# SamsungLabs/Metis

Hardware: NVIDIA B200
Metric: candidate plans evaluated/sec (higher is better)
Workload: dtype f64

## Files before the change

metis_b200/csrc/metis_coop.cuh:

```cuda
#pragma once

#include "metis_eval.cuh"

#ifdef METIS_HOST_STATS
extern "C" void metis_host_stats(int slot, long add);
#endif

namespace metis {

struct CoopMail {
    int m;
    int err;
    int flag;
    int pad;
    double val;
    double val2;
    int k;
    int s_top;
    int top_skip;
    int pad2;
};

struct OneLane {
    bool reverse = false;
// ... 605 lines not shown
                owner[layer] = (uint8_t)top;
                w.capa[top] = ntop;
                w.capa[nb] = nnb;
                if (top > nb) { int r = layer - 1; while (owner[r] != nb) --r; w.lastl[nb] = (uint16_t)r; }
                else          { int r = layer + 1; while (owner[r] != nb) ++r; w.first[nb] = (uint16_t)r; }
                if (w.cnt[top] == 0) { w.first[top] = (uint16_t)layer; w.lastl[top] = (uint16_t)layer; }
                else {
                    if (layer < (int)w.first[top]) w.first[top] = (uint16_t)layer;
                    if (layer > (int)w.lastl[top]) w.lastl[top] = (uint16_t)layer;
                }
                ++w.cnt[top];
                --w.cnt[nb];
            }
            x.sync();
        }
        x.mark(16);
        int carry = 0;
#pragma unroll 1
        for (int base = 0; base < S; base += x.width()) {
            const int s = base + x.lane();
            const int v = s < S ? (int)w.cnt[s] : 0;
            const int inc = x.incl_scan(v);
            if (s < S) w.part[s + 1] = (uint16_t)(carry + inc);
            carry += x.last_lane(inc);
        }
        if (x.leader()) w.part[0] = 0;
        x.sync();
        return METIS_FATAL_NONE;
    }

    MB_HD int adjust_performance_coop() {
        const int S = pd.S;
        const bool one_type = ONE || T.p.num_types == 1;
        double *ratio = reinterpret_cast<double *>(w.subw);
        double *mcap = ratio + MAXS / 2;
        static_assert(MAXL >= MAXS, "subw doubles as two S-sized fp64 arrays only when MAXL >= 2 * MAXS / 2");
        (void)mcap;
        x.sync();
        METIS_PAR(x, s, S) {
            const int a = one_type ? 0 : this->rank_start(s), b = a + this->group(s);
            const double c = w.perf[s], md = w.extra[s];
            const double mc = one_type ? T.type_memory[0] * (double)this->group(s) : this->memory_capacity(a, b);
            double av, adj;
            if (mc > md) {
                adj = c;
                av = (c * mc / md) - c;
            } else {
                av = 0.0;
                adj = c * (mc / md) * 0.9;
            }
            w.capa[s] = av;
            w.mstate[s] = adj;
            ratio[s] = (mc > md) ? 0.0 : (c - adj);
        }
        x.sync();
        if (x.leader()) {
            double need = 0.;
#pragma unroll 4
            for (int s = 0; s < S; ++s)
                if (w.capa[s] == 0.0 && ratio[s] != 0.0) need += ratio[s];
                else if (ratio[s] != 0.0) need += ratio[s];
            mail.val = need;
            mail.flag = seq_py_sum(w.capa, S) < need ? 1 : 0;
        }
        x.sync();
        if (mail.flag) return 1;
        METIS_PAR(x, s, S) w.extra[s] = 0.;
        x.sync();
        if (x.leader()) {
            double need = mail.val;
// ... 53 lines not shown
                const int rc = this->hetero_memory_demand(s, type0, md);
                if (rc) err = (double)rc + (double)aux * 256.0;
            }
            const double state = one_type ? T.type_memory[0] * (double)(1 << g) - md : this->memory_capacity(a, b) - md;
            w.extra[s] = md;
            w.capa[s] = state;
            w.mstate[s] = err;
            failed = failed || err != 0.0;
            oom = oom || state < 0;
        }
        failed = x.any(failed);
        oom = x.any(oom);
        if (failed) return -first_error(w.mstate, S);
        x.sync();
        if (!oom) {
            METIS_PAR(x, s, S) w.mstate[s] = w.capa[s];
            x.sync();
            return 1;
        }
        if (attempt >= 3) return 0;
        x.mark(21);
        const int rc = adjust_performance_coop();
        if (rc < 0) return rc;
        return rc == 1 ? 0 : 2;
    }

    MB_HD int get_cost_coop(double &cost_out) {
        const int per = T.p.devices_per_node;
        const int Lm = T.p.num_layers;
        const bool one_type = ONE || T.p.num_types == 1;
        const bool ubw = T.p.uniform_bw != 0;
        const int nstage = pd.label < pd.S ? pd.label : pd.S;
        if (T.p.q10_devices < T.p.total_devices && this->rank_start(nstage) > T.p.q10_devices) return 1;
        double *ppterm = reinterpret_cast<double *>(w.subw);
        bool bad = false;
        double max_len = -INFINITY, max_upd = -INFINITY, max_dp = -INFINITY;
        x.sync();
        METIS_PAR(x, s, nstage) {
            const int g = w.gcode[s], tpc = w.tpc[s];
            const int a = one_type ? 0 : this->rank_start(s), b = a + (1 << g);
            const int la = w.part[s], lb = w.part[s + 1];
            const int ldp = g - tpc;
            const int mbs = bs_total >> ldp;
            const int ta = one_type ? 0 : type_of_rank(T, pd.ns, a);
            const int tb = one_type ? 0 : type_of_rank(T, pd.ns, b - 1);
            double len = 0.0;
            if (ta == tb) {
                const int key = key_of(T, ta, tpc, mbs);
                if (key < 0) bad = true;
                else len = range_sum<SerialUniform>(T, kRangeLc, key, T.lc + (size_t)key * T.p.lpad, la, lb);
            } else if (this->hetero_exec_cost(a, b, 1 << ldp, tpc, la, lb, len)) {
                bad = true;
            }
            w.capa[s] = len;
            if (len > max_len) max_len = len;
            const double inv_tp = pow2_neg(tpc);
            double pp = 0.0;
            if (s < nstage - 1) {
                if (ubw) {
                    pp = (lb == Lm - 1) ? T.pp_vocab[mbs * T.p.num_tp + tpc] : T.pp_hidden[mbs];
                } else {
                    double act;
                    if (lb == Lm - 1)
                        act = (double)((int64_t)mbs * T.p.sequence_length * T.p.vocab_size) * inv_tp;
                    else
                        act = (double)((int64_t)mbs * T.p.sequence_length * T.p.hidden_size);
                    const int a2 = this->rank_start(s), b2 = this->rank_start(s + 2);
// ... 108 lines not shown
```

metis_b200/csrc/metis_eval.cuh:

```cuda
#pragma once

#include <stdint.h>
#include <string.h>
#include <math.h>

#include "../../include/metis_b200.h"

#if defined(__CUDACC__)
#define MB_HD __host__ __device__ __forceinline__
#define MB_HD_NOINLINE __host__ __device__ __noinline__
#else
#define MB_HD inline
#define MB_HD_NOINLINE inline
#endif

namespace metis {

template <class V>
MB_HD V list_load(const V *p) {
#if defined(__CUDA_ARCH__)
    return __ldcg(p);
#else
    return *p;
#endif
// ... 114 lines not shown
    unsigned mask;
    __device__ Lockstep() : mask(0xFFFFFFFFu) {}
    __device__ void converge() const { __syncwarp(mask); }
    __device__ void rejoin(bool p) { mask = __ballot_sync(0xFFFFFFFFu, p); }
};
#endif
struct SerialUniform : Serial {
    static constexpr bool kUniform = true;
};

constexpr uint64_t kOnes = 0x0101010101010101ULL;

constexpr uint16_t kBroke = 0x8000;
constexpr uint16_t kTaken = 0x4000;
constexpr uint16_t kPos = 0x3FFF;

template <int MAXS, int MAXL>
struct Scratch {
    static constexpr int kBlock = MAXS + 64;
    double perf[MAXS];
    double capa[MAXS];
    double mstate[MAXS];
    double extra[MAXS];
    uint16_t fe[MAXS];
    uint16_t first[MAXS], lastl[MAXS], cnt[MAXS];
    uint16_t part[MAXS + 1];
    uint16_t rs[MAXS + 1];
    uint8_t gcode[MAXS];
    uint8_t tpc[MAXS];
    uint8_t lstk[MAXS];
    uint8_t got[MAXS];
    uint8_t blk[kBlock];
    uint64_t ownerw[MAXL / 8 + 1];
    uint64_t subw[MAXL];
};

MB_HD double py_sum_range(const double *x, int a, int b) {
    if (a >= b) return 0.0;
    double f = 0.0 + x[a];
    double c = 0.0;
    for (int i = a + 1; i < b; ++i) {
        const double v = x[i];
        const double t = f + v;
        if (fabs(f) >= fabs(v)) c += (f - t) + v;
        else c += (v - t) + f;
        f = t;
    }
    if (c != 0.0 && isfinite(c)) f += c;
    return f;
}

MB_HD_NOINLINE double py_sum_range_compact(const double *x, int a, int b) {
    if (a >= b) return 0.0;
    double f = 0.0 + x[a];
    double c = 0.0;
#pragma unroll 1
    for (int i = a + 1; i < b; ++i) {
        const double v = x[i];
        const double t = f + v;
        if (fabs(f) >= fabs(v)) c += (f - t) + v;
        else c += (v - t) + f;
        f = t;
    }
    if (c != 0.0 && isfinite(c)) f += c;
    return f;
}

// ... 78 lines not shown
#pragma unroll 1
    for (int k = 0; k < nt; ++k)
        if (rank < end[k]) return typ[k];
    return typ[nt - 1];
}

MB_HD int type_of_q10(const Tables &T, int ns, int idx) {
    const int nt = T.p.num_types;
    const int32_t *end = T.q10_end + ns * nt;
    const uint8_t *typ = T.run_type + ns * nt;
#pragma unroll 1
    for (int k = 0; k < nt; ++k)
        if (idx < end[k]) return typ[k];
    return typ[nt - 1];
}

MB_HD int key_of(const Tables &T, int type, int tpc, int bs) {
    if (tpc >= T.p.num_tp || bs < 1 || bs > T.p.num_bs) return -1;
    return T.key_index[(type * T.p.num_tp + tpc) * T.p.num_bs + (bs - 1)];
}

template <int MAXS, int MAXL>
MB_HD int fwd_start(const Scratch<MAXS, MAXL> &w, int s) {
    if (s == 0) return 0;
    const uint16_t e = w.fe[s - 1];
    return (e & kPos) + ((e & kBroke) ? 1 : 0);
}

template <int MAXS, int MAXL>
MB_HD bool fwd_nonempty(const Scratch<MAXS, MAXL> &w, int s) {
    return (int)(w.fe[s] & kPos) > fwd_start(w, s);
}

MB_HD void sub_store(uint64_t *subw, int j, int stage) {
    reinterpret_cast<uint8_t *>(subw)[(j / kH) * 8 + (j % kH)] = (uint8_t)stage;
}

MB_HD int popc64(uint64_t v) {
#if defined(__CUDA_ARCH__)
    return __popcll(v);
#else
    return __builtin_popcountll(v);
#endif
}
MB_HD int ctz64(uint64_t v) {
#if defined(__CUDA_ARCH__)
    return __ffsll((long long)v) - 1;
#else
    return __builtin_ctzll(v);
#endif
}
MB_HD int popc32(uint32_t v) {
#if defined(__CUDA_ARCH__)
    return __popc(v);
#else
    return __builtin_popcount(v);
#endif
}
MB_HD int ctz32(uint32_t v) {
#if defined(__CUDA_ARCH__)
    return __ffs((int)v) - 1;
#else
    return __builtin_ctz(v);
#endif
}
MB_HD int clz32(uint32_t v) {
#if defined(__CUDA_ARCH__)
    return __clz((int)v);
#else
    return __builtin_clz(v);
// ... 31 lines not shown
    const int c0 = (int)(v & 0xFF), c1 = (int)((v >> 8) & 0xFF), c2 = (int)((v >> 16) & 0xFF);
    if (swar_count(v, c0) * 2 > kH) return c0;
    if (c1 != c0 && swar_count(v, c1) * 2 > kH) return c1;
    if (c2 != c1 && c2 != c0 && swar_count(v, c2) * 2 > kH) return c2;
    return (int)kDropped;
}

template <int MAXS, int MAXL, class X>
MB_HD int balance_run(const Tables &T, int S, Scratch<MAXS, MAXL> &w, const X &x) {
    const int L = T.p.num_layers;
    if (T.p.norm_len < L) return METIS_FATAL_INDEX;
    const double *dlay = T.dlay;
    const double *lc = T.norm_lc;
    const int N = kH * L;
    const int lim = (N - 1 - kH) > 0 ? (N - 1 - kH) : 0;
    const int last = S - 1;
    int broken = METIS_FATAL_NONE;

    x.sync();
#pragma unroll (X::kUniform ? 1 : 0)
    for (int s = x.lane(); s < S; s += x.width()) { w.capa[s] = w.perf[s]; w.got[s] = 0; w.cnt[s] = 0; }
    x.sync();

    x.mark(10);
    int k = 0, sTop = -1;
    bool topSkip = false;
    if (S > 1) {
        int s = 0, j = 0;
        double c = w.capa[0];
#pragma unroll (X::kUniform ? 1 : 0)
        for (int r = 0; r + 1 < L; ++r) {
            const double d = dlay[r];
            const int nsub = (r == L - 2) ? kH - 1 : kH;
            const int s_in = s;
            uint64_t v = 0;
#pragma unroll
            for (int q = 0; q < kH; ++q) {
                if (q < nsub) {
                    if (s < last) {
                        if (c > d) {
                            c -= d;
                            v |= (uint64_t)(uint32_t)s << (8 * q);
                        } else {
                            w.capa[s] = c;
                            w.fe[s] = (uint16_t)(j | kBroke);
                            ++s;
                            c = w.capa[s];
                        }
                    }
                    ++j;
                }
            }
            if (s_in < last) w.subw[r] = v;
        }
        if (s < last) {
            w.capa[s] = c;
            w.fe[s] = (uint16_t)lim;
#pragma unroll (X::kUniform ? 1 : 0)
            for (int t = s + 1; t < last; ++t) w.fe[t] = (uint16_t)lim;
            k = lim;
            sTop = s;
        } else {
            k = (w.fe[last - 1] & kPos) + 1;
            sTop = last - 1;
            topSkip = true;
        }
    }

    x.mark(11);
    x.converge();
    int m;
    {
        double c = w.capa[last];
        const double dl = dlay[L - 1];
#pragma unroll (X::kUniform ? 1 : 0)
        for (int i = 0; i < kH; ++i) c -= dl;
        m = N - kH;
        int sp = S - 2;
#pragma unroll (X::kUniform ? 1 : 0)
        while (m > 0) {
            const int j = m - 1;
            bool un = (j >= k);
            if (!un) {
#pragma unroll (X::kUniform ? 1 : 0)
                while (sp >= 0 && (!(w.fe[sp] & kBroke) || (int)(w.fe[sp] & kPos) > j)) --sp;
                un = (sp >= 0 && (int)(w.fe[sp] & kPos) == j);
// ... 19 lines not shown
            const int next_start = pos + ((e & kBroke) ? 1 : 0);
            if ((e & (kBroke | kTaken)) != kBroke) { start = next_start; continue; }
            const int j = pos;
            int lo = 0;
            if (pos > start) {
                lo = s;
            } else {
#pragma unroll (X::kUniform ? 1 : 0)
                for (int u = s;; --u) {
                    if (u < s) {
                        const int t = w.lstk[u];
                        const bool above = (t == last) || (fwd_nonempty(w, t) && fwd_start(w, t) > j);
                        if (!above) { lo = t; break; }
                    }
                    if (fwd_nonempty(w, u)) { lo = u; break; }
                    if (u == 0) break;
                }
            }
            int hi = s + 1;
            if (hi < last && !((int)(w.fe[hi] & kPos) > next_start && !w.got[hi])) {
                ++hi;
#pragma unroll (X::kUniform ? 1 : 0)
                while (hi < last && (!fwd_nonempty(w, hi) || w.got[hi])) ++hi;
            }
            if (lo > hi) { broken = METIS_FATAL_SCRATCH; hi = lo; }
            int pick = lo;
            double best = w.capa[lo];
#pragma unroll (X::kUniform ? 1 : 0)
            for (int t = lo + 1; t <= hi; ++t)
                if (w.capa[t] > best) { best = w.capa[t]; pick = t; }
            w.capa[pick] -= dlay[j / kH];
            w.lstk[s] = (uint8_t)pick;
            w.got[pick] = 1;
            sub_store(w.subw, j, pick);
            start = next_start;
        }
    }
    x.converge();
    int nblk = m - k;
    if (nblk > Scratch<MAXS, MAXL>::kBlock) { broken = METIS_FATAL_SCRATCH; nblk = Scratch<MAXS, MAXL>::kBlock; }
    {
        int below = -1;
#pragma unroll (X::kUniform ? 1 : 0)
        for (int t = 0; t < nblk; ++t) {
            const int j = k + t;
            int lo = 0;
            if (below >= 0) lo = below;
            else if (sTop >= 0) {
#pragma unroll (X::kUniform ? 1 : 0)
                for (int u = sTop;; --u) {
                    if (u < sTop || topSkip) {
                        const uint16_t eu = w.fe[u];
                        if ((eu & (kBroke | kTaken)) == kBroke) {
                            const int t2 = w.lstk[u];
                            if (t2 != last) { lo = t2; break; }
                        }
                    }
                    if (fwd_nonempty(w, u)) { lo = u; break; }
                    if (u == 0) break;
                }
            }
            int pick = lo;
            double best = w.capa[lo];
#pragma unroll (X::kUniform ? 1 : 0)
            for (int t2 = lo + 1; t2 <= last; ++t2)
                if (w.capa[t2] > best) { best = w.capa[t2]; pick = t2; }
            w.capa[pick] -= dlay[j / kH];
            w.blk[t] = (uint8_t)pick;
            if (pick != last) below = pick;
            sub_store(w.subw, j, pick);
        }
    }

    x.mark(13);
    x.converge();
    x.sync();
    int run_own = (int)kDropped, run_first = 0, run_len = 0;
#pragma unroll (X::kUniform ? 1 : 0)
    for (int r = x.lane(); r < L; r += x.width()) {
        const int nlow = m - kH * r;
        int own;
        if (nlow <= 0) {
            own = last;
        } else {
            uint64_t v = w.subw[r];
            if (nlow < kH) {
                const uint64_t mask = (1ULL << (8 * nlow)) - 1ULL;
                v = (v & mask) | (((uint64_t)last * kOnes) & ~mask);
            }
            v |= 0xFF00000000000000ULL;
            own = layer_owner(v, (T.p.corrected & METIS_FIX_Q5) != 0);
        }
        reinterpret_cast<uint8_t *>(w.ownerw)[r] = (uint8_t)own;
        {
            if (own == run_own) ++run_len;
            else {
                if (run_own != (int)kDropped) {
                    if (w.cnt[run_own] == 0) w.first[run_own] = (uint16_t)run_first;
                    w.lastl[run_own] = (uint16_t)(r - 1);
                    w.cnt[run_own] = (uint16_t)(w.cnt[run_own] + run_len);
                }
                run_own = own; run_first = r; run_len = 1;
            }
        }
    }
    if (run_own != (int)kDropped) {
        if (w.cnt[run_own] == 0) w.first[run_own] = (uint16_t)run_first;
        w.lastl[run_own] = (uint16_t)(L - 1);
        w.cnt[run_own] = (uint16_t)(w.cnt[run_own] + run_len);
    }
    x.sync();
    x.mark(14);
    x.converge();
    uint8_t *owner = reinterpret_cast<uint8_t *>(w.ownerw);
    x.sync();
#pragma unroll (X::kUniform ? 1 : 0)
    for (int s = x.lane(); s < S; s += x.width())
        w.capa[s] = w.cnt[s] ? w.perf[s] - range_sum<X>(T, kRangeNorm, 0, lc, w.first[s], (int)w.lastl[s] + 1) : w.perf[s];
    x.sync();

    x.mark(15);
    x.converge();
#pragma unroll (X::kUniform ? 1 : 0)
// ... 353 lines not shown
            if (key < 0) { aux = ((uint32_t)tpc << 16) | (uint32_t)bs; return METIS_FATAL_KEY_MEMORY; }
            demand += range_sum<SerialUniform>(T, kRangeMem, key, T.mem + (size_t)key * T.p.lpad, la, lb) * kMemCoef;
            return 0;
        }
        HSplit hs;
        const int rc = partition_data(T, pd.ns, a, b - a, 1 << (g - tpc), tpc, bs_total, hs, aux);
        if (rc) return rc;
        double worst = 0.0;
#pragma unroll 1
        for (int r = 0; r < hs.nruns; ++r)
#pragma unroll 1
            for (int v = 0; v < 2; ++v) {
                const int cntv = v ? hs.plus[r] : hs.n[r] - hs.plus[r];
                const int h = hs.base[r] + v;
                if (cntv <= 0 || h == 0) continue;
                double need = 0.0;
#pragma unroll 1
                for (int bit = 30; bit >= 0; --bit) {
                    const int piece = 1 << bit;
                    if (!(h & piece)) continue;
                    const int key = key_of(T, hs.type[r], tpc, piece);
                    if (key < 0) { aux = ((uint32_t)tpc << 16) | (uint32_t)piece; return METIS_FATAL_KEY_MEMORY; }
                    need += range_sum<SerialUniform>(T, kRangeMem, key, T.mem + (size_t)key * T.p.lpad, la, lb) * kMemCoef;
                }
                if (need > worst) worst = need;
            }
        demand += worst;
        return 0;
    }

    MB_HD_NOINLINE int adjust_performance() {
        const int S = pd.S;
        const bool one_type = ONE || T.p.num_types == 1;
        double *ratio = reinterpret_cast<double *>(w.subw);
        x.sync();
#pragma unroll (X::kUniform ? 1 : 0)
        for (int s = x.lane(); s < S; s += x.width()) {
            const int a = one_type ? 0 : rank_start(s), b = a + group(s);
            const double c = w.perf[s], md = w.extra[s];
            const double mc = one_type ? T.type_memory[0] * (double)group(s) : memory_capacity(a, b);
            double av, adj;
            if (mc > md) {
                adj = c;
                av = (c * mc / md) - c;
            } else {
                av = 0.0;
                adj = c * (mc / md) * 0.9;
            }
            w.capa[s] = av;
            w.mstate[s] = adj;
        }
        x.sync();
        double need = 0.;
        PySum avail_sum;
#pragma unroll (X::kUniform ? 1 : 0)
        for (int s = 0; s < S; ++s) {
            const int a = one_type ? 0 : rank_start(s);
            const double mc = one_type ? T.type_memory[0] * (double)group(s) : memory_capacity(a, a + group(s));
            if (!(mc > w.extra[s])) need += (w.perf[s] - w.mstate[s]);
            avail_sum.add(w.capa[s]);
        }
        if (avail_sum.result() < need) return 1;
        x.sync();
#pragma unroll (X::kUniform ? 1 : 0)
        for (int s = x.lane(); s < S; s += x.width()) w.extra[s] = 0.;
        x.sync();
        int guard = 0;
// ... 192 lines not shown

    MB_HD int get_cost(double &cost_out) {
        const int per = T.p.devices_per_node;
        const int Lm = T.p.num_layers;
        const bool one_type = ONE || T.p.num_types == 1;
        const bool ubw = T.p.uniform_bw != 0;
        const int nstage = pd.label < pd.S ? pd.label : pd.S;
        if (T.p.q10_devices < T.p.total_devices && rank_start(nstage) > T.p.q10_devices) return 1;
        x.sync();
#pragma unroll (X::kUniform ? 1 : 0)
        for (int s = x.lane(); s < nstage; s += x.width()) {
            const int g = w.gcode[s], tpc = w.tpc[s];
            const int a = one_type ? 0 : rank_start(s), b = a + (1 << g);
            const int la = w.part[s], lb = w.part[s + 1];
            const int ldp = g - tpc;
            const int ta = one_type ? 0 : type_of_rank(T, pd.ns, a);
            const int tb = one_type ? 0 : type_of_rank(T, pd.ns, b - 1);
            double len = 0.0, err = 0.0;
            if (ta == tb) {
                const int key = key_of(T, ta, tpc, bs_total >> ldp);
                if (key < 0) err = 1.0;
                else len = range_sum<X>(T, kRangeLc, key, T.lc + (size_t)key * T.p.lpad, la, lb);
            } else if (hetero_exec_cost(a, b, 1 << ldp, tpc, la, lb, len)) {
                err = 1.0;
            }
            w.capa[s] = len;
            w.extra[s] = err;
        }
        x.sync();
        bool bad = false;
#pragma unroll (X::kUniform ? 1 : 0)
        for (int s = x.lane(); s < nstage; s += x.width()) bad = bad || (w.extra[s] != 0.0);
        if (x.any(bad)) return 1;
        double *ppterm = reinterpret_cast<double *>(w.subw);
        double max_len = -INFINITY, max_upd = -INFINITY, max_dp = -INFINITY;
#pragma unroll (X::kUniform ? 1 : 0)
        for (int s = x.lane(); s < nstage; s += x.width()) {
            const int g = w.gcode[s], tpc = w.tpc[s];
            const int la = w.part[s], lb = w.part[s + 1];
            const int ldp = g - tpc;
            const int mbs = bs_total >> ldp;
            const double inv_tp = pow2_neg(tpc);
            if (w.capa[s] > max_len) max_len = w.capa[s];
            double pp = 0.0;
            if (s < nstage - 1) {
                if (ubw) {
                    pp = (lb == Lm - 1) ? T.pp_vocab[mbs * T.p.num_tp + tpc] : T.pp_hidden[mbs];
                } else {
                    double act;
                    if (lb == Lm - 1)
                        act = (double)((int64_t)mbs * T.p.sequence_length * T.p.vocab_size) * inv_tp;
                    else
                        act = (double)((int64_t)mbs * T.p.sequence_length * T.p.hidden_size);
                    const int a = rank_start(s), b2 = rank_start(s + 2);
                    pp = act / (bw_of_node_range(a / per, (b2 - 1) / per) * 1048576.0);
                }
            }
            ppterm[s] = pp;
            int ntr = lb - la;
            double params = 0.0;
            if (la == 0) { params += T.p.input_params * inv_tp; --ntr; }
            if (lb == Lm) { params += T.p.output_params * inv_tp; --ntr; }
            params += T.p.transformer_params * inv_tp * (double)ntr;
            double dpc;
            if (ubw) dpc = T.dpk[ldp] * params;
            else {
                const int dp = 1 << ldp;
// ... 185 lines not shown
```

metis_b200/csrc/metis_search.cu:

```cuda
#include <cuda_runtime.h>
#include <cooperative_groups.h>
#include <stdint.h>
#include <stdio.h>
#include <stdlib.h>
#include <string.h>

#include "metis_eval.cuh"
#include "metis_coop.cuh"
#include "metis_trace.cuh"
#include "metis_rows.cuh"

namespace cg = cooperative_groups;

namespace metis {

#ifndef METIS_THREADS
#define METIS_THREADS 256
#endif
#ifndef METIS_MIN_BLOCKS
#define METIS_MIN_BLOCKS 3
#endif
#ifndef METIS_MIN_BLOCKS_BIG
#define METIS_MIN_BLOCKS_BIG METIS_MIN_BLOCKS
#endif
#ifndef METIS_MIN_BLOCKS_BIG_ONE
#define METIS_MIN_BLOCKS_BIG_ONE (METIS_MIN_BLOCKS + 1)
#endif
constexpr int kThreads = METIS_THREADS;
constexpr int kMaxS = METIS_MAX_STAGES;
constexpr int kMaxL = METIS_MAX_LAYERS;
constexpr int kSmemBlobMax = 160 * 1024;

static thread_local char g_err[256] = "";
static thread_local cudaEvent_t g_ev_before = nullptr, g_ev_after = nullptr;

static int cuda_fail(cudaError_t e, const char *what) {
    snprintf(g_err, sizeof(g_err), "%s: %s", what, cudaGetErrorString(e));
    return METIS_E_CUDA;
}
static int arg_fail(const char *what) {
    snprintf(g_err, sizeof(g_err), "%s", what);
    return METIS_E_ARG;
}
int fail_cuda(cudaError_t e, const char *what) { return cuda_fail(e, what); }
int fail_arg(const char *what) { return arg_fail(what); }

struct BlobLayout {
    uint32_t total;
    uint32_t key, lc, mem, exec_full, fb, norm, derived, tmem, bwf, bwm, runt, rune, q10e;
    uint32_t rsum, rsum_bytes;
};

static uint32_t align16(uint32_t v) { return (v + 15u) & ~15u; }

static BlobLayout make_layout(const MetisProblem &p) {
    BlobLayout l;
    uint32_t o = 0;
    const uint32_t nkey = (uint32_t)p.num_types * p.num_tp * p.num_bs;
    l.key = o;       o = align16(o + nkey * 2);
    l.lc = o;        o = align16(o + (uint32_t)p.num_keys * p.lpad * 8);
    l.mem = o;       o = align16(o + (uint32_t)p.num_keys * p.lpad * 8);
// ... 3 lines not shown
    l.derived = o;   o = align16(o + (uint32_t)derived_layout(p).total * 8);
    l.tmem = o;      o = align16(o + (uint32_t)p.num_types * 8);
    l.bwf = o;       o = align16(o + (uint32_t)p.num_types * 8);
    l.bwm = o;       o = align16(o + (uint32_t)p.num_types * 8);
    l.runt = o;      o = align16(o + (uint32_t)p.num_node_sequences * p.num_types);
    l.rune = o;      o = align16(o + (uint32_t)p.num_node_sequences * p.num_types * 4);
    l.q10e = o;      o = align16(o + (uint32_t)p.num_node_sequences * p.num_types * 4);
    l.total = o;
    const uint64_t n = (uint64_t)p.num_layers + 1;
    l.rsum = (o + 127u) & ~127u;
    l.rsum_bytes = (uint32_t)((uint64_t)(2 * p.num_keys + 1) * n * n * 8);
    return l;
}

__device__ __forceinline__ Tables make_tables(const MetisProblem &p, const BlobLayout &l, const uint8_t *base,
                                              const uint8_t *gblob = nullptr) {
    Tables T;
    T.p = p;
    T.rsum = gblob ? reinterpret_cast<const double *>(gblob + l.rsum) : nullptr;
    T.key_index = reinterpret_cast<const int16_t *>(base + l.key);
    T.lc = reinterpret_cast<const double *>(base + l.lc);
    T.mem = reinterpret_cast<const double *>(base + l.mem);
    T.exec_full = reinterpret_cast<const double *>(base + l.exec_full);
    T.fb_sync = reinterpret_cast<const double *>(base + l.fb);
    T.norm_lc = reinterpret_cast<const double *>(base + l.norm);
    bind_derived(T, reinterpret_cast<const double *>(base + l.derived));
    T.type_memory = reinterpret_cast<const double *>(base + l.tmem);
    T.bw_first = reinterpret_cast<const double *>(base + l.bwf);
    T.bw_min = reinterpret_cast<const double *>(base + l.bwm);
    T.run_type = base + l.runt;
    T.run_end = reinterpret_cast<const int32_t *>(base + l.rune);
    T.q10_end = reinterpret_cast<const int32_t *>(base + l.q10e);
    return T;
}

__device__ __forceinline__ void copy_bytes(uint8_t *dst, const void *src, uint32_t n, uint32_t tid, uint32_t nthr) {
    const uint8_t *s = static_cast<const uint8_t *>(src);
    for (uint32_t i = tid; i < n; i += nthr) dst[i] = s[i];
}

__global__ void pack_tables_kernel(MetisProblem p, BlobLayout l, uint8_t *blob) {
    const uint32_t tid = blockIdx.x * blockDim.x + threadIdx.x, nthr = gridDim.x * blockDim.x;
    const uint32_t nkey = (uint32_t)p.num_types * p.num_tp * p.num_bs;
    copy_bytes(blob + l.key, p.key_index, nkey * 2, tid, nthr);
    copy_bytes(blob + l.lc, p.layer_compute, (uint32_t)p.num_keys * p.lpad * 8, tid, nthr);
    copy_bytes(blob + l.mem, p.layer_memory, (uint32_t)p.num_keys * p.lpad * 8, tid, nthr);
    copy_bytes(blob + l.exec_full, p.exec_full, (uint32_t)p.num_keys * 8, tid, nthr);
    copy_bytes(blob + l.fb, p.fb_sync, (uint32_t)p.num_keys * 8, tid, nthr);
    copy_bytes(blob + l.norm, p.norm_lc, (uint32_t)p.norm_len * 8, tid, nthr);
    copy_bytes(blob + l.tmem, p.type_memory, (uint32_t)p.num_types * 8, tid, nthr);
    copy_bytes(blob + l.bwf, p.type_bw_first, (uint32_t)p.num_types * 8, tid, nthr);
    copy_bytes(blob + l.bwm, p.type_bw_min, (uint32_t)p.num_types * 8, tid, nthr);
    copy_bytes(blob + l.runt, p.ns_run_type, (uint32_t)p.num_node_sequences * p.num_types, tid, nthr);
    copy_bytes(blob + l.rune, p.ns_run_end, (uint32_t)p.num_node_sequences * p.num_types * 4, tid, nthr);
    copy_bytes(blob + l.q10e, p.ns_q10_end, (uint32_t)p.num_node_sequences * p.num_types * 4, tid, nthr);
    double *derived = reinterpret_cast<double *>(blob + l.derived);
    const DerivedLayout d = derived_layout(p);
    for (uint32_t i = tid; i < (uint32_t)d.total; i += nthr)
        derived[i] = derive_entry(p, d, p.norm_lc, p.exec_full, p.type_bw_first, (int)i);
}

__global__ void __launch_bounds__(128)
range_sums_kernel(MetisProblem p, BlobLayout l, uint8_t *blob) {
    const int L = p.num_layers;
    const long long i = (long long)blockIdx.x * blockDim.x + threadIdx.x;
    if (i >= (long long)range_sum_tables(p) * L) return;
// ... 237 lines not shown
        if (lane == __ffs(peers) - 1) atomicAdd(&ls.ctl[kCtlHist + k], (unsigned int)__popc(peers));
        if (lane == __ffs(peers3) - 1) atomicAdd(&ls.ctl[kCtlHist3 + key], (unsigned int)__popc(peers3));
    }
}

__global__ void __launch_bounds__(256)
het_scatter_kernel(const SearchLists ls) {
    __shared__ unsigned int s_base[160];
    const unsigned int n = ls.ctl[0];
    const bool bulk = (long long)n >= ls.bulk_min;
    const int hist = bulk ? kCtlHist : kCtlHist3, cursor = bulk ? kCtlCursor : kCtlCursor3;
    if (threadIdx.x == 0) {
        unsigned int acc = 0;
        for (int k = 127; k >= 0; --k) { s_base[k] = acc; acc += ls.ctl[hist + k]; }
    }
    __syncthreads();
    const long long span = (long long)gridDim.x * blockDim.x;
    const long long upto = (((long long)n + 31) / 32) * 32;
    for (long long pos = (long long)blockIdx.x * blockDim.x + threadIdx.x; pos < upto; pos += span) {
        const bool live = pos < (long long)n;
        uint4 e = make_uint4(0, 0, 0, 0);
        if (live) e = ls.a[pos];
        const int k = !live ? -1 : bulk ? (int)(e.w & 0xFF) : (int)((e.y >> 8) & 0x7F);
        const unsigned int peers = __match_any_sync(0xFFFFFFFFu, k);
        const int leader = __ffs(peers) - 1, me = threadIdx.x & 31;
        unsigned int at = 0;
        if (live && me == leader) at = atomicAdd(&ls.ctl[cursor + k], (unsigned int)__popc(peers));
        at = __shfl_sync(0xFFFFFFFFu, at, leader);
        if (live) ls.b[(long long)s_base[k] + at + __popc(peers & ((1u << me) - 1u))] = e;
    }
}

template <int MAXS, int MAXL, bool ONE>
__global__ void __launch_bounds__(kThreads, (MAXS <= 64 ? METIS_MIN_BLOCKS : ONE ? METIS_MIN_BLOCKS_BIG_ONE : METIS_MIN_BLOCKS_BIG))
het_first_kernel(const __grid_constant__ MetisProblem p, const __grid_constant__ MetisPlanSpace sp,
                 const __grid_constant__ BlobLayout lay, const uint8_t *__restrict__ blob, const int use_smem,
                 const __grid_constant__ DeviceOut out, const SearchLists ls, const int best_slot) {
    extern __shared__ __align__(128) uint8_t smem[];
    __shared__ uint64_t mbar;
    DeviceSink sink(out);
    const unsigned int n = ls.ctl[0];
    if ((long long)n >= ls.bulk_min) {
        const uint8_t *base = blob;
        if (use_smem) {
            stage_blob_tma(smem, blob, lay.total, &mbar);
            base = smem;
        }
        const Tables T = make_tables(p, lay, base, blob);
        Scratch<MAXS, MAXL> w;
        const int lane = threadIdx.x & 31;
        for (;;) {
            unsigned int fetched = 0;
            if (lane == 0) fetched = atomicAdd(&ls.ctl[1], 1u);
            const long long b0 = 32LL * __shfl_sync(0xFFFFFFFFu, fetched, 0);
            if (b0 >= (long long)n) break;
            const long long pos = b0 + lane;
            PlanDesc pd;
            const bool has = pos < (long long)n;
            uint4 e = make_uint4(0, 0, 0, 0);
            if (has) { e = ls.b[pos]; decode_entry(sp, e, pd); }
            int hint = 0, start = 1;
            const bool cont = first_task<MAXS, MAXL, ONE, Lockstep>(T, w, sink, has, pd, hint, start);
            const unsigned m = __ballot_sync(0xFFFFFFFFu, cont);
            if (m) {
                const int leader = __ffs(m) - 1;
                unsigned int at = 0;
                if (lane == leader) at = atomicAdd(&ls.ctl[2], (unsigned int)__popc(m));
                at = __shfl_sync(0xFFFFFFFFu, at, leader);
                if (cont) {
                    const unsigned key = hint < 0 ? 0u : (hint > 127 ? 127u : (unsigned)hint);
                    const unsigned int c = at + __popc(m & ((1u << lane) - 1u));
                    if (start == 2) {
                        if (c < ls.save_cap) {
                            for (int s = 0; s < pd.S; ++s) ls.perf[(size_t)s * ls.save_cap + c] = w.perf[s];
                        } else start = 1;
                    }
                    e.y = 1u | ((unsigned)start << 1) | (key << 8);
                    ls.a[c] = e;
                    atomicAdd(&ls.ctl[kCtlHist2 + key], 1u);
                }
            }
        }
    }
    finish_block(sink, out, best_slot + blockIdx.x);
}

__global__ void __launch_bounds__(256)
het_order_kernel(const SearchLists ls) {
    __shared__ unsigned int s_base[128];
    if ((long long)ls.ctl[0] < ls.bulk_min) return;
    const unsigned int n = ls.ctl[2];
    if (threadIdx.x == 0) {
        unsigned int acc = 0;
        for (int k = 127; k >= 0; --k) { s_base[k] = acc; acc += ls.ctl[kCtlHist2 + k]; }
    }
    __syncthreads();
    const long long span = (long long)gridDim.x * blockDim.x;
    for (long long pos = (long long)blockIdx.x * blockDim.x + threadIdx.x; pos < (long long)n; pos += span) {
        const uint4 e = ls.a[pos];
        const unsigned key = (e.y >> 8) & 0x7Fu;
        const unsigned int to = s_base[key] + atomicAdd(&ls.ctl[kCtlCursor2 + key], 1u);
        ls.b[to] = e;
        ls.src[to] = (unsigned int)pos;
    }
}

#ifdef METIS_PROFILE_PHASES
__device__ long long g_mark_acc[64];
#endif
struct WarpCoop {
#ifdef METIS_PROFILE_PHASES
// ... 91 lines not shown
        return dkey_inv(kmax(dkey(v), mine));
    }
    __device__ __noinline__ int incl_scan(int v) const {
        const int lane = threadIdx.x & 31;
#pragma unroll
        for (int d = 1; d < 32; d <<= 1) {
            const int u = __shfl_up_sync(0xFFFFFFFFu, v, d);
            if (lane >= d) v += u;
        }
        return v;
    }
    __device__ int last_lane(int v) const { return __shfl_sync(0xFFFFFFFFu, v, 31); }
};

template <int MAXS, int MAXL>
struct alignas(16) ChainScratch {
    Scratch<MAXS, MAXL> w;
    CoopMail mail;
};

template <int MAXS, int MAXL, bool ONE>
__global__ void __launch_bounds__(512, 2)
het_chain_kernel(const __grid_constant__ MetisProblem p, const __grid_constant__ MetisPlanSpace sp,
                 const __grid_constant__ BlobLayout lay, const uint8_t *__restrict__ blob, const int use_smem,
                 const unsigned int scratch_off, const __grid_constant__ DeviceOut out, const SearchLists ls,
                 const int best_slot) {
    extern __shared__ __align__(128) uint8_t smem[];
    __shared__ uint64_t mbar;
    const uint8_t *base = blob;
    if (use_smem) {
        stage_blob_tma(smem, blob, lay.total, &mbar);
        base = smem;
    }
    const Tables T = make_tables(p, lay, base, blob);
    DeviceSink sink(out);
    const int lane = threadIdx.x & 31;
    sink.leader = lane == 0;
    ChainScratch<MAXS, MAXL> *cs = reinterpret_cast<ChainScratch<MAXS, MAXL> *>(smem + scratch_off) + (threadIdx.x >> 5);
    const unsigned int n_adm = ls.ctl[0];
    const bool bulk = (long long)n_adm >= ls.bulk_min;
    const uint4 *list = ls.b;
    const unsigned int n = bulk ? ls.ctl[2] : n_adm;
    WarpCoop lanes;
    CoopEvaluator<MAXS, MAXL, WarpCoop, ONE> ev(T, cs->w, cs->mail, lanes);
    for (;;) {
        unsigned int i = 0;
        if (lane == 0) i = atomicAdd(&ls.ctl[3], 1u);
        i = __shfl_sync(0xFFFFFFFFu, i, 0);
        if (i >= n) break;
        const uint4 e = __ldcg(&list[i]);
        PlanDesc pd;
        decode_entry(sp, e, pd);
        lanes.mark(1);
        const int start = (e.y & 1u) ? (int)((e.y >> 1) & 3u) : 0;
        const double *perf = nullptr;
        if (start == 2) perf = ls.perf + __ldcg(&ls.src[i]);
        ev.run_chain(pd, sink, start, perf, (size_t)ls.save_cap);
        lanes.mark(0);
    }
    while (WarpCoop::block_or(0)) {}
    sink.leader = true;
    if (lane != 0) { sink.n_part = sink.n_run = sink.n_key = 0; }
    finish_block(sink, out, best_slot + blockIdx.x);
}

__global__ void het_finalize_kernel(const MetisRecord *block_best, int nblocks, const unsigned long long *counters,
                                    const unsigned int *ctl, MetisSearchSummary *summary) {
// ... 294 lines not shown
        int best_warps = 0;
        for (int threads = 64; threads <= 512; threads *= 2) {
            if (forced && threads != ((forced + 31) & ~31)) continue;
            const unsigned int off = chain_smem_tables ? blob_pad : 0u;
            const size_t dyn = off + (size_t)(threads / 32) * per_warp;
            if (dyn > (size_t)smem_optin) continue;
            if (dyn > 48 * 1024) {
                e = cudaFuncSetAttribute(chain, cudaFuncAttributeMaxDynamicSharedMemorySize, (int)dyn);
                if (e != cudaSuccess) { cudaGetLastError(); continue; }
            }
            int per_sm = 0;
            e = cudaOccupancyMaxActiveBlocksPerMultiprocessor(&per_sm, chain, threads, dyn);
            if (e != cudaSuccess || per_sm < 1) { cudaGetLastError(); continue; }
            const int warps = per_sm * threads / 32;
            if (warps > best_warps) { best_warps = warps; chain_threads = threads; chain_per_sm = per_sm; chain_dyn = dyn; chain_off = off; }
        }
        if (chain_threads == 0) chain_smem_tables = 0;
    }
    if (chain_threads == 0) return arg_fail("chain kernel does not fit this device (shared memory)");
    if (chain_dyn > 48 * 1024) {
        e = cudaFuncSetAttribute(chain, cudaFuncAttributeMaxDynamicSharedMemorySize, (int)chain_dyn);
        if (e != cudaSuccess) return cuda_fail(e, "cudaFuncSetAttribute(chain)");
    }
    int64_t chain_grid = (int64_t)sms * chain_per_sm;

    auto first = het_first_kernel<MAXS, MAXL, ONE>;
    int first_smem_tables = (int)lay.total <= blob_max && blob_pad <= (unsigned int)smem_optin;
    size_t first_dyn = first_smem_tables ? blob_pad : 0;
    if (first_dyn > 48 * 1024) {
        e = cudaFuncSetAttribute(first, cudaFuncAttributeMaxDynamicSharedMemorySize, (int)first_dyn);
        if (e != cudaSuccess) { cudaGetLastError(); first_smem_tables = 0; first_dyn = 0; }
    }
    int first_per_sm = 0;
    e = cudaOccupancyMaxActiveBlocksPerMultiprocessor(&first_per_sm, first, kThreads, first_dyn);
    if (e != cudaSuccess || first_per_sm < 1) return cuda_fail(e, "occupancy query (bulk round)");
    int64_t first_grid = (int64_t)sms * first_per_sm;
    if (first_grid + chain_grid > kMaxBlocks) return arg_fail("grid exceeds the per-block best table");

    ls.bulk_min = sh.reserved > 0 ? (long long)sh.reserved : 12LL * chain_grid * (chain_threads / 32);

    if (g_ev_before) cudaEventRecord(g_ev_before, stream);
    if (slots > 0) {
        const int64_t admit_blocks = (slots + 255) / 256;
        if (admit_blocks > 0x7FFFFFFFLL) return arg_fail("too many plans for one launch");
        het_admit_kernel<<<(unsigned)admit_blocks, 256, 0, stream>>>(s_arg, sh, (long long)slots, p_arg.gbs, p_arg.max_bs,
                                                                     p_arg.max_tp, ls);
        int64_t scatter_blocks = (slots + 255) / 256;
        if (scatter_blocks > 8LL * sms) scatter_blocks = 8LL * sms;
        het_scatter_kernel<<<(unsigned)scatter_blocks, 256, 0, stream>>>(ls);
        first<<<(unsigned)first_grid, kThreads, first_dyn, stream>>>(p_arg, s_arg, lay, ws.blob, first_smem_tables, out, ls, 0);
        het_order_kernel<<<(unsigned)(2 * sms), 256, 0, stream>>>(ls);
        chain<<<(unsigned)chain_grid, chain_threads, chain_dyn, stream>>>(p_arg, s_arg, lay, ws.blob, chain_smem_tables,
                                                                         chain_off, out, ls, (int)first_grid);
        e = cudaGetLastError();
        if (e != cudaSuccess) return cuda_fail(e, "search kernels");
    }
    if (g_ev_after) cudaEventRecord(g_ev_after, stream);
    g_ev_before = g_ev_after = nullptr;
    het_finalize_kernel<<<1, 256, 0, stream>>>(ws.block_best, (int)(slots > 0 ? first_grid + chain_grid : 0), ws.counters,
                                               ws.ctl, ws.summary);
    e = cudaGetLastError();
    if (e != cudaSuccess) return cuda_fail(e, "het_finalize_kernel");
    return METIS_OK;
}

extern "C" {

int metis_het_search(const MetisProblem *problem, const MetisPlanSpace *space, const MetisShard *shard,
                     MetisRecord *records, int64_t capacity, uint8_t *detail, int32_t detail_stride,
                     void *workspace, int64_t workspace_bytes, MetisSearchSummary *summary, void *stream_) {
    int rc = check_problem(problem);
    if (rc) return rc;
    if (!space || !shard || !workspace || !summary) return arg_fail("NULL argument");
    if (shard->world < 1 || shard->rank < 0 || shard->rank >= shard->world || shard->tile < 32 || shard->tile % 32)
        return arg_fail("bad shard (tile must be a positive multiple of 32)");
    if (space->num_plans > 0xFFFFFFF0LL) return arg_fail("more than 2^32 plans");
    if (space->max_stage < 1 || space->max_stage > METIS_MAX_STAGES) return arg_fail("max_stage out of range (METIS_MAX_STAGES)");
    if (space->num_div < 1 || space->num_div > 256) return arg_fail("more than 256 divisors of gbs");
    if (problem->num_node_sequences < 1 || problem->num_node_sequences > 256)
        return arg_fail("more than 256 node sequences (geometry word)");
    if (space->rows_bytes < 0 || space->rows_bytes > 0xFFFFFFFFLL) return arg_fail("row tables must be smaller than 4 GiB (geometry word)");
    if (detail && detail_stride < 3 * space->max_stage + 1) return arg_fail("detail_stride too small (3 * max_stage + 1)");
    if (capacity < 0 || (capacity > 0 && !records)) return arg_fail("records/capacity mismatch");
// ... 134 lines not shown
```

Before: 195.0 million.

## Drop per-layer sub-owner buffer, share Tables in smem, retune big-stage block size

```diff
diff --git a/metis_b200/csrc/metis_coop.cuh b/metis_b200/csrc/metis_coop.cuh
--- a/metis_b200/csrc/metis_coop.cuh
+++ b/metis_b200/csrc/metis_coop.cuh
@@ -661,10 +661,7 @@
     MB_HD int adjust_performance_coop() {
         const int S = pd.S;
         const bool one_type = ONE || T.p.num_types == 1;
-        double *ratio = reinterpret_cast<double *>(w.subw);
-        double *mcap = ratio + MAXS / 2;
-        static_assert(MAXL >= MAXS, "subw doubles as two S-sized fp64 arrays only when MAXL >= 2 * MAXS / 2");
-        (void)mcap;
+        double *ratio = w.term;
         x.sync();
         METIS_PAR(x, s, S) {
             const int a = one_type ? 0 : this->rank_start(s), b = a + this->group(s);
@@ -784,7 +781,7 @@
         const bool ubw = T.p.uniform_bw != 0;
         const int nstage = pd.label < pd.S ? pd.label : pd.S;
         if (T.p.q10_devices < T.p.total_devices && this->rank_start(nstage) > T.p.q10_devices) return 1;
-        double *ppterm = reinterpret_cast<double *>(w.subw);
+        double *ppterm = w.term;
         bool bad = false;
         double max_len = -INFINITY, max_upd = -INFINITY, max_dp = -INFINITY;
         x.sync();
diff --git a/metis_b200/csrc/metis_eval.cuh b/metis_b200/csrc/metis_eval.cuh
--- a/metis_b200/csrc/metis_eval.cuh
+++ b/metis_b200/csrc/metis_eval.cuh
@@ -170,7 +170,7 @@
     uint8_t got[MAXS];
     uint8_t blk[kBlock];
     uint64_t ownerw[MAXL / 8 + 1];
-    uint64_t subw[MAXL];
+    double term[MAXS];
 };
 
 MB_HD double py_sum_range(const double *x, int a, int b) {
@@ -315,10 +315,6 @@
     return (int)(w.fe[s] & kPos) > fwd_start(w, s);
 }
 
-MB_HD void sub_store(uint64_t *subw, int j, int stage) {
-    reinterpret_cast<uint8_t *>(subw)[(j / kH) * 8 + (j % kH)] = (uint8_t)stage;
-}
-
 MB_HD int popc64(uint64_t v) {
 #if defined(__CUDA_ARCH__)
     return __popcll(v);
@@ -416,15 +412,12 @@
         for (int r = 0; r + 1 < L; ++r) {
             const double d = dlay[r];
             const int nsub = (r == L - 2) ? kH - 1 : kH;
-            const int s_in = s;
-            uint64_t v = 0;
 #pragma unroll
             for (int q = 0; q < kH; ++q) {
                 if (q < nsub) {
                     if (s < last) {
                         if (c > d) {
                             c -= d;
-                            v |= (uint64_t)(uint32_t)s << (8 * q);
                         } else {
                             w.capa[s] = c;
                             w.fe[s] = (uint16_t)(j | kBroke);
@@ -435,7 +428,6 @@
                     ++j;
                 }
             }
-            if (s_in < last) w.subw[r] = v;
         }
         if (s < last) {
             w.capa[s] = c;
@@ -521,7 +513,6 @@
             w.capa[pick] -= dlay[j / kH];
             w.lstk[s] = (uint8_t)pick;
             w.got[pick] = 1;
-            sub_store(w.subw, j, pick);
             start = next_start;
         }
     }
@@ -557,7 +548,6 @@
             w.capa[pick] -= dlay[j / kH];
             w.blk[t] = (uint8_t)pick;
             if (pick != last) below = pick;
-            sub_store(w.subw, j, pick);
         }
     }
 
@@ -565,19 +555,29 @@
     x.converge();
     x.sync();
     int run_own = (int)kDropped, run_first = 0, run_len = 0;
+    int slot = -1, nxt = 0;
+    uint16_t e = 0;
 #pragma unroll (X::kUniform ? 1 : 0)
     for (int r = x.lane(); r < L; r += x.width()) {
-        const int nlow = m - kH * r;
+        const int j0 = kH * r;
         int own;
-        if (nlow <= 0) {
+        if (j0 >= m) {
             own = last;
         } else {
-            uint64_t v = w.subw[r];
-            if (nlow < kH) {
-                const uint64_t mask = (1ULL << (8 * nlow)) - 1ULL;
-                v = (v & mask) | (((uint64_t)last * kOnes) & ~mask);
-            }
-            v |= 0xFF00000000000000ULL;
+            uint64_t v = 0xFF00000000000000ULL;
+#pragma unroll
+            for (int q = 0; q < kH; ++q) {
+                const int j = j0 + q;
+                int st;
+                if (j >= m) st = last;
+                else if (j >= k) st = (j - k < nblk) ? (int)w.blk[j - k] : last;
+                else {
+#pragma unroll (X::kUniform ? 1 : 0)
+                    while (nxt <= j) { ++slot; e = w.fe[slot]; nxt = (int)(e & kPos) + ((e & kBroke) ? 1 : 0); }
+                    st = (nxt - 1 == j && (e & kBroke)) ? (int)w.lstk[slot] : slot;
+                }
+                v |= (uint64_t)(uint32_t)st << (8 * q);
+            }
             own = layer_owner(v, (T.p.corrected & METIS_FIX_Q5) != 0);
         }
         reinterpret_cast<uint8_t *>(w.ownerw)[r] = (uint8_t)own;
@@ -997,7 +997,7 @@
     MB_HD_NOINLINE int adjust_performance() {
         const int S = pd.S;
         const bool one_type = ONE || T.p.num_types == 1;
-        double *ratio = reinterpret_cast<double *>(w.subw);
+        double *ratio = w.term;
         x.sync();
 #pragma unroll (X::kUniform ? 1 : 0)
         for (int s = x.lane(); s < S; s += x.width()) {
@@ -1256,7 +1256,7 @@
 #pragma unroll (X::kUniform ? 1 : 0)
         for (int s = x.lane(); s < nstage; s += x.width()) bad = bad || (w.extra[s] != 0.0);
         if (x.any(bad)) return 1;
-        double *ppterm = reinterpret_cast<double *>(w.subw);
+        double *ppterm = w.term;
         double max_len = -INFINITY, max_upd = -INFINITY, max_dp = -INFINITY;
 #pragma unroll (X::kUniform ? 1 : 0)
         for (int s = x.lane(); s < nstage; s += x.width()) {
diff --git a/metis_b200/csrc/metis_search.cu b/metis_b200/csrc/metis_search.cu
--- a/metis_b200/csrc/metis_search.cu
+++ b/metis_b200/csrc/metis_search.cu
@@ -20,13 +20,18 @@
 #ifndef METIS_MIN_BLOCKS
 #define METIS_MIN_BLOCKS 3
 #endif
+#ifndef METIS_THREADS_BIG
+#define METIS_THREADS_BIG 384
+#endif
 #ifndef METIS_MIN_BLOCKS_BIG
-#define METIS_MIN_BLOCKS_BIG METIS_MIN_BLOCKS
+#define METIS_MIN_BLOCKS_BIG 2
 #endif
 #ifndef METIS_MIN_BLOCKS_BIG_ONE
 #define METIS_MIN_BLOCKS_BIG_ONE (METIS_MIN_BLOCKS + 1)
 #endif
 constexpr int kThreads = METIS_THREADS;
+template <int MAXS, bool ONE>
+constexpr int first_threads() { return (MAXS <= 64 || ONE) ? METIS_THREADS : METIS_THREADS_BIG; }
 constexpr int kMaxS = METIS_MAX_STAGES;
 constexpr int kMaxL = METIS_MAX_LAYERS;
 constexpr int kSmemBlobMax = 160 * 1024;
@@ -96,6 +101,14 @@
     T.run_end = reinterpret_cast<const int32_t *>(base + l.rune);
     T.q10_end = reinterpret_cast<const int32_t *>(base + l.q10e);
     return T;
+}
+
+__device__ __forceinline__ const Tables &block_tables(const MetisProblem &p, const BlobLayout &l, const uint8_t *base,
+                                                      const uint8_t *gblob) {
+    __shared__ Tables s_tables;
+    if (threadIdx.x == 0) s_tables = make_tables(p, l, base, gblob);
+    __syncthreads();
+    return s_tables;
 }
 
 __device__ __forceinline__ void copy_bytes(uint8_t *dst, const void *src, uint32_t n, uint32_t tid, uint32_t nthr) {
@@ -399,7 +412,7 @@
 }
 
 template <int MAXS, int MAXL, bool ONE>
-__global__ void __launch_bounds__(kThreads, (MAXS <= 64 ? METIS_MIN_BLOCKS : ONE ? METIS_MIN_BLOCKS_BIG_ONE : METIS_MIN_BLOCKS_BIG))
+__global__ void __launch_bounds__((first_threads<MAXS, ONE>()), (MAXS <= 64 ? METIS_MIN_BLOCKS : ONE ? METIS_MIN_BLOCKS_BIG_ONE : METIS_MIN_BLOCKS_BIG))
 het_first_kernel(const __grid_constant__ MetisProblem p, const __grid_constant__ MetisPlanSpace sp,
                  const __grid_constant__ BlobLayout lay, const uint8_t *__restrict__ blob, const int use_smem,
                  const __grid_constant__ DeviceOut out, const SearchLists ls, const int best_slot) {
@@ -413,7 +426,7 @@
             stage_blob_tma(smem, blob, lay.total, &mbar);
             base = smem;
         }
-        const Tables T = make_tables(p, lay, base, blob);
+        const Tables &T = block_tables(p, lay, base, blob);
         Scratch<MAXS, MAXL> w;
         const int lane = threadIdx.x & 31;
         for (;;) {
@@ -424,8 +437,7 @@
             const long long pos = b0 + lane;
             PlanDesc pd;
             const bool has = pos < (long long)n;
-            uint4 e = make_uint4(0, 0, 0, 0);
-            if (has) { e = ls.b[pos]; decode_entry(sp, e, pd); }
+            if (has) decode_entry(sp, ls.b[pos], pd);
             int hint = 0, start = 1;
             const bool cont = first_task<MAXS, MAXL, ONE, Lockstep>(T, w, sink, has, pd, hint, start);
             const unsigned m = __ballot_sync(0xFFFFFFFFu, cont);
@@ -442,8 +454,7 @@
                             for (int s = 0; s < pd.S; ++s) ls.perf[(size_t)s * ls.save_cap + c] = w.perf[s];
                         } else start = 1;
                     }
-                    e.y = 1u | ((unsigned)start << 1) | (key << 8);
-                    ls.a[c] = e;
+                    ls.a[c] = make_entry(pd.ordinal, 1u | ((unsigned)start << 1) | (key << 8), pd.geo);
                     atomicAdd(&ls.ctl[kCtlHist2 + key], 1u);
                 }
             }
@@ -601,7 +612,7 @@
         stage_blob_tma(smem, blob, lay.total, &mbar);
         base = smem;
     }
-    const Tables T = make_tables(p, lay, base, blob);
+    const Tables &T = block_tables(p, lay, base, blob);
     DeviceSink sink(out);
     const int lane = threadIdx.x & 31;
     sink.leader = lane == 0;
@@ -962,7 +973,7 @@
         if (e != cudaSuccess) { cudaGetLastError(); first_smem_tables = 0; first_dyn = 0; }
     }
     int first_per_sm = 0;
-    e = cudaOccupancyMaxActiveBlocksPerMultiprocessor(&first_per_sm, first, kThreads, first_dyn);
+    e = cudaOccupancyMaxActiveBlocksPerMultiprocessor(&first_per_sm, first, first_threads<MAXS, ONE>(), first_dyn);
     if (e != cudaSuccess || first_per_sm < 1) return cuda_fail(e, "occupancy query (bulk round)");
     int64_t first_grid = (int64_t)sms * first_per_sm;
     if (first_grid + chain_grid > kMaxBlocks) return arg_fail("grid exceeds the per-block best table");
@@ -978,7 +989,7 @@
         int64_t scatter_blocks = (slots + 255) / 256;
         if (scatter_blocks > 8LL * sms) scatter_blocks = 8LL * sms;
         het_scatter_kernel<<<(unsigned)scatter_blocks, 256, 0, stream>>>(ls);
-        first<<<(unsigned)first_grid, kThreads, first_dyn, stream>>>(p_arg, s_arg, lay, ws.blob, first_smem_tables, out, ls, 0);
+        first<<<(unsigned)first_grid, first_threads<MAXS, ONE>(), first_dyn, stream>>>(p_arg, s_arg, lay, ws.blob, first_smem_tables, out, ls, 0);
         het_order_kernel<<<(unsigned)(2 * sms), 256, 0, stream>>>(ls);
         chain<<<(unsigned)chain_grid, chain_threads, chain_dyn, stream>>>(p_arg, s_arg, lay, ws.blob, chain_smem_tables,
                                                                          chain_off, out, ls, (int)first_grid);
```

Measured after the change: 205.0 million, median of 6. +5.2%, better.
